# YiwenShaoStephen/mergeNet

Hardware: AMD Instinct MI355X
Metric: merged Mpixels/sec at 1024x2048 (speculative fast path; proven path: value_proven_path) (higher is better)
Workload: dtype f32

## Files before the change

### include/mergenet_hip.h

```cpp
#ifndef MERGENET_HIP_H_
#define MERGENET_HIP_H_

#include <stddef.h>
#include <stdint.h>

#ifdef __cplusplus
extern "C" {
#endif

#define MN_MAX_OFFSETS 32
#define MN_MAX_CLASSES 127

enum mn_status {
  MN_OK = 0,
  MN_ERR_ARGUMENT = -1,
  MN_ERR_OFFSETS = -2,
  MN_ERR_NO_DEVICE = -3,
  MN_ERR_CAPACITY = -4,
  MN_ERR_NO_BACKGROUND = -10,
  MN_ERR_INTERNAL = -20,
  MN_ERR_UNPROVEN = -30
};

enum mn_variant {
// ... 92 lines not shown
int mn_segment_finish(mn_context* ctx, mn_stats* stats);

int mn_sweep_time_device(mn_context* ctx, const float* const* d_class_pred, const float* const* d_adj_pred,
                         int n_inputs, int class_dim, int offset_dim, int img_width, int img_height,
                         int num_classes, const int* offset_list, const mn_options* opts, void* stream, int reps,
                         float* us_per_launch);

int mn_segment_exact_batch(mn_context** ctxs, int count, const float* const* d_class_pred, int class_dim,
                           const float* const* d_adj_pred, int offset_dim, int img_width, int img_height,
                           int num_classes, const int* offset_list, int* const* d_mask,
                           int* const* d_object_class, int* const* d_partition, const mn_options* opts,
                           void* stream, mn_stats* stats);

int mn_score_device(mn_context* ctx, const float* d_class_pred, int class_dim,
                    const float* d_adj_pred, int offset_dim, int img_width, int img_height,
                    int num_classes, const int* offset_list, const mn_options* opts, void* stream,
                    unsigned char* d_cls_out, unsigned long long* d_best_out, float* ms_class_pass,
                    float* ms_edge_pass);

int mn_sweep_device(mn_context* ctx, const float* d_class_pred, int class_dim, const float* d_adj_pred,
                    int offset_dim, int img_width, int img_height, int num_classes, const int* offset_list,
                    const mn_options* opts, void* stream, unsigned* d_bits_out, float* d_neg_out,
                    unsigned char* d_cls_out, int* d_gsum_out, double* logsum_out, int* info_out);

int mn_exact_phase_a_device(mn_context* ctx, const float* d_class_pred, int class_dim,
                            const float* d_adj_pred, int offset_dim, int img_width, int img_height,
                            int num_classes, const int* offset_list, const mn_options* opts, void* stream,
                            unsigned char* d_cls_out, float* d_oml_out, float* d_prio_out);

int mn_segment_device_t(mn_context* ctx, const void* d_class_pred, int class_dim, const void* d_adj_pred,
                        int offset_dim, int dtype, int img_width, int img_height, int num_classes,
                        const int* offset_list, int* d_mask, int* d_object_class, int* d_partition,
                        const mn_options* opts, void* stream, mn_stats* stats);
int mn_segment_launch_t(mn_context* ctx, const void* d_class_pred, int class_dim, const void* d_adj_pred,
                        int offset_dim, int dtype, int img_width, int img_height, int num_classes,
                        const int* offset_list, int* d_mask, int* d_object_class, int* d_partition,
                        const mn_options* opts, void* stream);
int mn_segment_exact_batch_t(mn_context** ctxs, int count, const void* const* d_class_pred, int class_dim,
                             const void* const* d_adj_pred, int offset_dim, int dtype, int img_width,
                             int img_height, int num_classes, const int* offset_list, int* const* d_mask,
                             int* const* d_object_class, int* const* d_partition, const mn_options* opts,
                             void* stream, mn_stats* stats);
int mn_score_device_t(mn_context* ctx, const void* d_class_pred, int class_dim, const void* d_adj_pred,
                      int offset_dim, int dtype, int img_width, int img_height, int num_classes,
                      const int* offset_list, const mn_options* opts, void* stream, unsigned char* d_cls_out,
                      unsigned long long* d_best_out, float* ms_class_pass, float* ms_edge_pass);
// ... 68 lines not shown
```

### mergenet_amd/csrc/mergenet_hip.hip

```cpp
#include <hip/hip_runtime.h>
#include <hip/hip_ext.h>

#include <math.h>
#include <stdio.h>
#include <stdlib.h>
#include <string.h>
#include <time.h>

#include "../../include/mergenet_hip.h"
#include "mn_device.h"
#include "mn_kernels_score.h"
#include "mn_kernels_merge.h"
#include "mn_kernels_finish.h"
#include "mn_kernels_output.h"
#include "mn_kernels_prepare.h"
#include "mn_kernels_cc.h"
#include "mn_kernels_tail.h"
#include "mn_kernels_exact.h"
#include "mn_kernels_reforder.h"

#define MN_NSCALARS 16
#define MN_STAT_BYTES ((((sizeof(Counters) + 15) & ~(size_t)15)) + MN_NSCALARS * sizeof(int) + 4 * sizeof(double))

#define MN_MAX_SUBROUNDS 64
// ... 61 lines not shown
  HashTab T;
  int* block_count;
  double* partial;
  Counters* cnt;
  int* scalars;
  unsigned* gmax;
  unsigned* touch;
  unsigned* h_touch;
  float* theta;
  int* progress;
  u64* bg_key;
  double* lp_out;
  Counters* h_cnt;
  int* h_scalars;
  double* h_lp;
  size_t cc_sum_lds, oc_lds;
  unsigned char* statblk;
  unsigned char* h_statblk;
  int *cc_tcount, *cc_lcount;
  unsigned* cc_bits;
  int* cc_roots;
  int cc_sign_blocks;
  unsigned* cc_negbits;
  size_t cc_cap_max;
  hipEvent_t ev[12];
  struct Pending {
    int active;
    int rc;
    Queued queued;
    ImageCall call;
    mn_stats stats;
  } pend;
  hipEvent_t ev_done;
  struct Replay {
    int state;
    int capturing;
    unsigned char key[256];
    size_t key_bytes;
    hipGraph_t gA, gB;
    hipGraphExec_t eA, eB;
    hipStream_t cap;
    Queued queued;
  } replay;
  hipStream_t side;
  hipEvent_t ev_fork;
  ImgParams last_params;
// ... 289 lines not shown
  if (hipSetDevice(device) != hipSuccess) { g_last_status = MN_ERR_NO_DEVICE; return NULL; }
  mn_context* c = static_cast<mn_context*>(calloc(1, sizeof(mn_context)));
  if (!c) { g_last_status = MN_ERR_INTERNAL; return NULL; }
  c->device = device;
  c->maxH = max_height; c->maxW = max_width; c->maxC = max_classes; c->maxO = max_offsets;
  c->N = (size_t)max_height * max_width;
  c->Rmax = c->N * (size_t)max_offsets;
  c->cap_full = next_pow2(c->Rmax + c->Rmax / 4 + 1024);
  if (ctx_alloc(c) != MN_OK) { mn_destroy(c); return NULL; }
  g_last_status = MN_OK;
  return c;
}

extern "C" void mn_destroy(mn_context* c) {
  if (!c) return;
  if (getenv("MN_TRACE_HOST") && g_host_n[1] > 0) {
    fprintf(stderr, "host: %lld launches %.1f us each; %lld read-backs: waiting for the image %.1f us, the rest %.1f us each\n",
            g_host_n[0], g_host_us[0] / (double)(g_host_n[0] ? g_host_n[0] : 1), g_host_n[1],
            g_host_us[1] / (double)g_host_n[1], g_host_us[2] / (double)g_host_n[1]);
    g_host_n[0] = g_host_n[1] = 0; g_host_us[0] = g_host_us[1] = g_host_us[2] = 0.0;
  }
  (void)hipSetDevice(c->device);
  void* dev[] = {c->ocls, c->cls0, c->lpvalid, c->matched, c->pruned, c->osize, c->parent, c->mate, c->root,
                 c->label, c->mapbuf, c->lpsum, c->lp_acc, c->ball, c->bsub, c->fin_lists, c->cc_tcount, c->cc_lcount, c->cc_bits, c->cc_roots, c->cc_negbits,
                 c->block_count, c->wire_counts, c->partial, c->statblk,
                 c->bg_key, c->gmax, c->touch, c->theta, c->progress, c->d_class, c->d_same, c->d_mask, c->d_objcls, c->d_part};
  for (size_t i = 0; i < sizeof(dev) / sizeof(dev[0]); i++)
    if (dev[i]) (void)hipFree(dev[i]);
  x_free(c);
  r_free(c);
  if (c->xw.d_P) (void)hipFree(c->xw.d_P);
  if (c->xw.d_X) (void)hipFree(c->xw.d_X);
  if (c->rw.d_S) (void)hipFree(c->rw.d_S);
  free_records(c);
  if (c->h_statblk) (void)hipHostFree(c->h_statblk);
  if (c->h_touch) (void)hipHostFree(c->h_touch);
  for (int i = 0; i < 12; i++)
    if (c->ev[i]) (void)hipEventDestroy(c->ev[i]);
  if (c->ev_done) (void)hipEventDestroy(c->ev_done);
  if (c->ev_fork) (void)hipEventDestroy(c->ev_fork);
  if (c->side) (void)hipStreamDestroy(c->side);
  if (c->replay.eA) (void)hipGraphExecDestroy(c->replay.eA);
  if (c->replay.eB) (void)hipGraphExecDestroy(c->replay.eB);
  if (c->replay.gA) (void)hipGraphDestroy(c->replay.gA);
  if (c->replay.gB) (void)hipGraphDestroy(c->replay.gB);
  if (c->replay.cap) (void)hipStreamDestroy(c->replay.cap);
  free(c);
}

extern "C" size_t mn_workspace_bytes(const mn_context* c) { return c ? c->bytes : 0; }

static int ensure_fast(mn_context* c) {
  if (c->lp_acc) return MN_OK;
  const size_t N = c->N;
  MN_HIP(dev_alloc(c, &c->lp_acc, N * (size_t)c->maxC));
  MN_HIP(dev_alloc(c, &c->ball, N));
  MN_HIP(dev_alloc(c, &c->bsub, N));
  MN_HIP(dev_alloc(c, &c->cc_bits, N));
  MN_HIP(dev_alloc(c, &c->cc_roots, N));
  MN_HIP(dev_alloc(c, &c->cc_negbits, N + 16));
  return MN_OK;
}

static void drop_replay_graphs(mn_context::Replay& rp) {
  if (rp.eA) { (void)hipGraphExecDestroy(rp.eA); rp.eA = nullptr; }
  if (rp.eB) { (void)hipGraphExecDestroy(rp.eB); rp.eB = nullptr; }
  if (rp.gA) { (void)hipGraphDestroy(rp.gA); rp.gA = nullptr; }
  if (rp.gB) { (void)hipGraphDestroy(rp.gB); rp.gB = nullptr; }
  rp.state = 0;
}

static int ensure_general(mn_context* c) {
  if (c->gen_ready) return MN_OK;
  MN_HIP(hipDeviceSynchronize());
  free_records(c);
  if (alloc_records(c, c->cap_full) != MN_OK) return MN_ERR_NO_DEVICE;
  c->cap = c->cap_full;
  c->gen_ready = 1;
  c->cc_clean = 0;
  drop_replay_graphs(c->replay);
  return MN_OK;
}

static int check_args(const mn_context* c, const ImageCall& call) {
  const int W = call.W, H = call.H, num_classes = call.num_classes, offset_dim = call.offset_dim;
  const int* offs = call.offs;
  if (!c || !call.has_offsets) return MN_ERR_ARGUMENT;
  if (W <= 0 || H <= 0 || num_classes <= 0 || offset_dim <= 0 || call.class_dim < num_classes)
    return MN_ERR_ARGUMENT;
  if (num_classes > MN_MAX_CLASSES || offset_dim > MN_MAX_OFFSETS) return MN_ERR_ARGUMENT;
  if ((size_t)W * H > c->N || num_classes > c->maxC || offset_dim > c->maxO) return MN_ERR_CAPACITY;
  if (call.opts.variant != MN_VARIANT_CSEGMENT && call.opts.variant != MN_VARIANT_PYSEGMENTER)
// ... 245 lines not shown
  } while (0)
  if (P.dtype == MN_DTYPE_F32) {
    if (px == 4) launch_sign<4, MN_DTYPE_F32>(c, P, st, cls, lean_cls);
    else launch_sign<1, MN_DTYPE_F32>(c, P, st, false, false);
  } else if (px == 8) MN_SWEEP_DT(8);
  else if (px == 4) MN_SWEEP_DT(4);
  else { cls = false; lean_cls = false; MN_SWEEP_DT(1); }
#undef MN_SWEEP_DT
}

template <int PX>
static void launch_cc_hook(mn_context* c, const ImgParams& P, hipStream_t st, unsigned kmask,
                           const unsigned* hook_bits = nullptr, hipEvent_t hook_done = nullptr) {
  const int N = P.N, ngroups = (N + PX - 1) / PX;
  const dim3 gx(8 * ((grid_for(ngroups, 256) + 7) / 8));
  if (hook_done)
    hipExtLaunchKernelGGL(mn_cc_hook<PX>, gx, dim3(256), 0, st, nullptr, hook_done, 0, P,
                          hook_bits ? hook_bits : (const unsigned*)c->cc_bits, c->parent, kmask);
  else
    hipLaunchKernelGGL(mn_cc_hook<PX>, gx, dim3(256), 0, st, P, hook_bits ? hook_bits : (const unsigned*)c->cc_bits,
                       c->parent, kmask);
}

enum CcUse {
  CC_WAITED,
  CC_QUEUED_COMPACT,
  CC_QUEUED_TAIL,
  CC_CORES
};

static int run_components(mn_context* c, const ImgParams& P, hipStream_t& st, CcUse use) {
  const bool wait = use == CC_WAITED, with_ball = use == CC_WAITED;
  const bool with_compact = use == CC_WAITED || use == CC_QUEUED_COMPACT;
  const bool fork_before_sums = use == CC_QUEUED_TAIL, cores = use == CC_CORES;
  const int N = P.N;
  ObjState S = obj_state(c);
  const dim3 b(256);
  const bool four = P.W % 4 == 0;
  int kh = -1, kv = -1, dv = 0;
  for (int k = 0; k < P.O; k++) {
    if (kh < 0 && P.di[k] == 0 && P.dj[k] == 1) kh = k;
    if (kv < 0 && P.dj[k] == 0 && (P.di[k] == 1 || P.di[k] == -1)) { kv = k; dv = P.di[k]; }
  }
  const bool few_events = (c->debug_flags & 2) != 0;
  const bool lean = (c->debug_flags & 16) != 0;
  const dim3 tiles((P.W + 63) / 64, (P.H + MN_CC_TILE_ROWS - 1) / MN_CC_TILE_ROWS);
  const int px = sweep_px(c, P);
  const bool sweep4 = px >= 4;
  const size_t sign_blocks = grid_for((size_t)(N / px), MN_CC_SIGN_THREADS);
  c->cc_sign_blocks = (int)(sign_blocks * (MN_CC_SIGN_THREADS / 64));
  int* clsmin = c->root;
  int* clsmax = c->mapbuf;
  const bool fused_cls = sweep4;
  const bool lean_cls = fused_cls && !cores;
  launch_sweep(c, P, st, px, fused_cls, lean_cls);
  if (!few_events && !c->ext_events) MN_HIP(hipEventRecord(c->ev[10], st));
  const unsigned* lbits = c->cc_bits;
  unsigned kshort = 0u;
  if (cores) {
    if (!fused_cls) {
      const unsigned blocks = grid_for((size_t)(N >> 2) > 0 ? (size_t)(N >> 2) : 1, 256);
      hipLaunchKernelGGL(mn_class_pass, dim3(blocks), dim3(256), 0, st, P, c->cls0);
    }
    unsigned* bits2 = reinterpret_cast<unsigned*>(c->label);
    for (int k = 0; k < P.O; k++)
      if (c->core_radius < 0 || (abs(P.di[k]) <= c->core_radius && abs(P.dj[k]) <= c->core_radius)) kshort |= 1u << k;
    hipLaunchKernelGGL(mn_core_clean, dim3(grid_for(N, 256)), b, 0, st, P, (const unsigned*)c->cc_bits,
                       (const unsigned char*)c->cls0, c->pruned, kshort);
    hipLaunchKernelGGL(mn_core_bits, dim3(grid_for(N, 256)), b, 0, st, P, (const unsigned char*)c->pruned,
                       (const unsigned*)c->cc_bits, (const unsigned char*)c->cls0, bits2);
    lbits = bits2;
  }
  hipStream_t real = st;
  if (c->replay.capturing) {
    MN_HIP(hipStreamBeginCapture(c->replay.cap, hipStreamCaptureModeThreadLocal));
    st = c->replay.cap;
  }
  unsigned kmask = P.O >= 32 ? 0xFFFFFFFFu : ((1u << P.O) - 1u);
  const bool fork_ext = fork_before_sums && c->ext_events && !c->replay.capturing;
  bool fork_by_hook = false;
  hipLaunchKernelGGL(mn_cc_tiles, tiles, dim3(MN_CC_TILE_ROWS * 64), 0, st, P, lbits, c->parent, kh, kv, dv,
                     c->osize, c->lp_acc, clsmin, clsmax, c->matched);
  if (kh >= 0 || kv >= 0) {
    hipLaunchKernelGGL(mn_cc_borders, tiles, dim3(128), 0, st, P, lbits, c->parent, kh, kv, dv);
    if (kh >= 0) kmask &= ~(1u << kh);
    if (kv >= 0) kmask &= ~(1u << kv);
  }
  hipLaunchKernelGGL(mn_cc_flatten, dim3(grid_for((size_t)(N >> 2) > 0 ? (size_t)(N >> 2) : 1, 256)), b, 0, st, N, c->parent);
  fork_by_hook = fork_ext && kmask;
  if (kmask) {
    if (four) launch_cc_hook<4>(c, P, st, kmask, lbits, fork_by_hook ? c->ev_fork : nullptr);
    else launch_cc_hook<1>(c, P, st, kmask, lbits, fork_by_hook ? c->ev_fork : nullptr);
  }
  if (c->replay.capturing) {
    MN_HIP(hipStreamEndCapture(c->replay.cap, &c->replay.gA));
    MN_HIP(hipGraphInstantiate(&c->replay.eA, c->replay.gA, nullptr, nullptr, 0));
    MN_HIP(hipGraphLaunch(c->replay.eA, real));
    st = real;
  }
  HashTab T = c->T;
  T.mask = (unsigned)(c->cc_cap - 1);
  if (!few_events && !lean) MN_HIP(hipEventRecord(c->ev[7], st));
  if (fork_before_sums) {
    if (!fork_by_hook) MN_HIP(hipEventRecord(c->ev_fork, st));
    MN_HIP(hipStreamWaitEvent(c->side, c->ev_fork, 0));
    st = c->side;
    if (c->replay.capturing) {
      MN_HIP(hipStreamBeginCapture(c->replay.cap, hipStreamCaptureModeThreadLocal));
      st = c->replay.cap;
    }
  }
  if (!few_events && !lean) MN_HIP(hipEventRecord(c->ev[11], st));
  {
    const size_t lds = (size_t)MN_CC_SUM_SLOTS * (P.C + 1) * sizeof(u64);
    if (lds > c->cc_sum_lds) {
      MN_HIP(hipFuncSetAttribute(reinterpret_cast<const void*>(mn_cc_class_sums),
// ... 1210 lines not shown
  HostBuf<double> hp(sign_waves * 2);
  if (!hp.ok()) return MN_ERR_INTERNAL;
  MN_HIP(hipMemcpyAsync(hp, c->partial, sign_waves * 2 * sizeof(double), hipMemcpyDeviceToHost, st));
  MN_HIP(hipMemcpyAsync(c->h_scalars, c->scalars, MN_NSCALARS * sizeof(int), hipMemcpyDeviceToHost, st));
  MN_HIP(hipStreamSynchronize(st));
  double t = 0.0;
  for (size_t b = 0; b < sign_waves; b++) t += hp[2 * b];
  if (logsum_out) *logsum_out = t;
  if (info_out) { info_out[0] = px; info_out[1] = fused_cls ? 1 : 0; info_out[2] = c->h_scalars[6]; }
  MN_HIP(hipGetLastError());
  g_last_status = MN_OK;
  return MN_OK;
}

extern "C" int mn_sweep_device(mn_context* c, const float* d_class_pred, int class_dim,
                               const float* d_adj_pred, int offset_dim, int W, int H, int num_classes,
                               const int* offset_list, const mn_options* opts, void* stream,
                               unsigned* d_bits_out, float* d_neg_out, unsigned char* d_cls_out,
                               int* d_gsum_out, double* logsum_out, int* info_out) {
  return mn_sweep_device_t(c, d_class_pred, class_dim, d_adj_pred, offset_dim, MN_DTYPE_F32, W, H, num_classes,
                           offset_list, opts, stream, d_bits_out, d_neg_out, d_cls_out, d_gsum_out, logsum_out, info_out);
}

extern "C" int mn_sweep_time_device_t(mn_context* c, const void* const* d_class_pred, const void* const* d_adj_pred,
                                      int dtype, int n_inputs, int class_dim, int offset_dim, int W, int H,
                                      int num_classes, const int* offset_list, const mn_options* opts, void* stream,
                                      int reps, float* us_per_launch) {
  const bool ok = d_class_pred && d_adj_pred && n_inputs >= 1 && reps >= 1 && us_per_launch;
  ImageCall call = {ok ? d_class_pred[0] : nullptr, ok ? d_adj_pred[0] : nullptr, dtype, class_dim, offset_dim, W, H, num_classes};
  image_call(&call, offset_list, opts, stream);
  ImgParams P;
  const int rc = begin_call(c, call, ok, nullptr, &P);
  if (rc != MN_OK) return rc;
  hipStream_t st = static_cast<hipStream_t>(stream);
  if (ensure_fast(c) != MN_OK) return MN_ERR_NO_DEVICE;
  c->debug_flags = call.opts.debug_flags | 2;
  c->ext_events = 0;
  c->cc_clean = 0;
  MN_HIP(hipMemsetAsync(c->scalars, 0, MN_NSCALARS * sizeof(int), st));
  for (int phase = 0; phase < 2; phase++) {
    const int n = phase == 0 ? (reps + 9) / 10 : reps;
    if (phase == 1) MN_HIP(hipEventRecord(c->ev[0], st));
    for (int i = 0; i < n; i++) {
      call.d_class = d_class_pred[i % n_inputs]; call.d_adj = d_adj_pred[i % n_inputs];
      fill_params(&P, call);
      launch_sweep(c, P, st, sweep_px(c, P), true, true);
// ... 372 lines not shown
```

### mergenet_amd/csrc/mn_kernels_cc.h

```cpp
#pragma once

static_assert(MN_MAX_OFFSETS <= 32, "edge masks are 32-bit words: one bit per offset");

#include "mn_device.h"
#include "mn_kernels_merge.h"

#define MN_LP_FIX 16777216.0

__device__ __forceinline__ int mn_cc_find(int* __restrict__ parent, int x) {
  int p = parent[x];
  while (p != x) {
    const int g = parent[p];
    if (g != p) parent[x] = g;
    x = p;
    p = g;
  }
  return x;
}

struct __attribute__((packed, aligned(4))) mn_int4u { int x, y, z, w; };
__device__ __forceinline__ int4 mn_ld_int4_unaligned(const int* __restrict__ p) {
  const mn_int4u t = *reinterpret_cast<const mn_int4u*>(p);
  return make_int4(t.x, t.y, t.z, t.w);
}
// ... 363 lines not shown

__device__ __forceinline__ void mn_cc_wave_union(int* __restrict__ parent, bool want, int a, int b) {
  const int lane = threadIdx.x & 63;
  u64 todo = __ballot(want);
  const u64 key = mn_key(a, b);
  while (todo) {
    const int first = __ffsll((long long)todo) - 1;
    const u64 k0v = ((u64)(unsigned)__shfl((int)(key >> 32), first) << 32) |
                    (u64)(unsigned)__shfl((int)(key & 0xFFFFFFFFull), first);
    const bool mine = want && key == k0v;
    if (lane == first) {
      while (a != b) {
        if (a < b) { const int t = a; a = b; b = t; }
        const int old = atomicMin(&parent[a], b);
        if (old == a) break;
        a = mn_cc_find(parent, old);
        b = mn_cc_find(parent, b);
      }
    }
    todo &= ~__ballot(mine);
  }
}

__global__ __launch_bounds__(128) void mn_cc_borders(ImgParams P, const unsigned* __restrict__ bits,
                                                     int* __restrict__ parent, int kh, int kv, int dv) {
  const int lane = threadIdx.x & 63, wave = threadIdx.x >> 6;
  const int r0 = (int)blockIdx.y * MN_CC_TILE_ROWS, c0 = (int)blockIdx.x * 64;
  int p = -1, q = -1;
  if (wave == 0) {
    const int r = r0 + lane, c = c0 + 63;
    if (kh >= 0 && lane < MN_CC_TILE_ROWS && r < P.H && c + 1 < P.W) {
      p = r * P.W + c;
      if ((bits[p] >> kh) & 1u) q = p + 1;
    }
  } else {
    const int r = dv > 0 ? r0 + MN_CC_TILE_ROWS - 1 : r0, c = c0 + lane;
    if (kv >= 0 && r < P.H && r + dv >= 0 && r + dv < P.H && c < P.W) {
      p = r * P.W + c;
      if ((bits[p] >> kv) & 1u) q = p + dv * P.W;
    }
  }
  int a = 0, b = 0;
  bool want = false;
  if (q >= 0) {
    a = mn_cc_find(parent, p);
    b = mn_cc_find(parent, q);
    want = a != b;
  }
  mn_cc_wave_union(parent, want, a, b);
}

__global__ __launch_bounds__(256) void mn_cc_flatten(int N, int* __restrict__ parent) {
  const int i = blockIdx.x * blockDim.x + threadIdx.x;
  const int n4 = N >> 2;
  if (i < n4) {
    int4 r = *reinterpret_cast<const int4*>(parent + 4 * (size_t)i);
    int4 o = r;
    int x = r.x; while (parent[x] != x) x = parent[x]; o.x = x;
    if (r.y == r.x) o.y = o.x; else { x = r.y; while (parent[x] != x) x = parent[x]; o.y = x; }
    if (r.z == r.x) o.z = o.x; else { x = r.z; while (parent[x] != x) x = parent[x]; o.z = x; }
    if (r.w == r.x) o.w = o.x; else { x = r.w; while (parent[x] != x) x = parent[x]; o.w = x; }
    if (o.x != r.x || o.y != r.y || o.z != r.z || o.w != r.w)
      *reinterpret_cast<int4*>(parent + 4 * (size_t)i) = o;
  }
  if (i < N - (n4 << 2)) {
    const int p = (n4 << 2) + i;
    int x = p; while (parent[x] != x) x = parent[x];
    parent[p] = x;
  }
}

template <int PX>
// ... 46 lines not shown
      }
    }
#pragma unroll
    for (int g = 0; g < G; g++) {
      const int k = k0 + g;
      if (k >= P.O) break;
      if (__ballot((any >> k) & 1u) == 0) continue;
#pragma unroll
      for (int j = 0; j < PX; j++) {
        bool want = false;
        int a = 0, bb = 0;
        if (((b[j] & kmask) >> k) & 1u) {
          if (rq[g][j] != own[j]) {
            const int q = p0 + j + P.di[k] * P.W + P.dj[k];
            a = mn_cc_find(parent, p0 + j);
            bb = mn_cc_find(parent, q);
            want = a != bb;
          }
        }
        mn_cc_wave_union(parent, want, a, bb);
      }
    }
  }
}

__global__ __launch_bounds__(256) void mn_core_clean(ImgParams P, const unsigned* __restrict__ bits,
                                                     const unsigned char* __restrict__ cls0,
                                                     unsigned char* __restrict__ clean, unsigned kshort) {
  const int p = blockIdx.x * blockDim.x + threadIdx.x;
  if (p >= P.N) return;
  const int r = p / P.W, c = p - r * P.W;
  const unsigned b = bits[p];
  const unsigned char mine = cls0[p];
  bool ok = true;
  for (int k = 0; k < P.O; k++) {
    if (!((kshort >> k) & 1u)) continue;
    const int di = P.di[k], dj = P.dj[k];
    if (r + di >= 0 && r + di < P.H && c + dj >= 0 && c + dj < P.W) {
      const int q = p + di * P.W + dj;
      ok = ok && ((b >> k) & 1u) && cls0[q] == mine;
    }
    if (r - di >= 0 && r - di < P.H && c - dj >= 0 && c - dj < P.W) {
      const int q = p - di * P.W - dj;
      ok = ok && ((bits[q] >> k) & 1u) && cls0[q] == mine;
    }
  }
// ... 675 lines not shown
```

### mergenet_amd/segmenter.py

```python

from __future__ import annotations

import ctypes
import os
import threading
from collections import namedtuple
from typing import List, Optional, Sequence, Tuple

import numpy as np

_HERE = os.path.dirname(os.path.abspath(__file__))
LIB_PATH = os.environ.get("MN_LIB") or os.path.join(_HERE, "libmergenet_hip.so")

MN_VARIANT_CSEGMENT = 0
MN_VARIANT_PYSEGMENTER = 1
MN_MODE_AUTO, MN_MODE_EXACT, MN_MODE_ROUNDS, MN_MODE_COMPONENTS = 0, 1, 2, 3
MN_ERR_NO_BACKGROUND = -10
MN_ERR_UNPROVEN = -30
MN_DEBUG_GENERIC_EDGE_PASS, MN_DEBUG_NO_EVENTS, MN_DEBUG_NO_CORES = 1, 2, 4
MN_DEBUG_LEAN_EVENTS, MN_DEBUG_REPLAY = 16, 32
MN_DEBUG_SWEEP16_4PX = 256
MN_DTYPE_F32, MN_DTYPE_F16, MN_DTYPE_BF16 = 0, 1, 2
MN_ERR_ARGUMENT = -1
MN_PROVE_ALWAYS, MN_PROVE_BY_MODE, MN_PROVE_NEVER = 1, 0, -1
# ... 21 lines not shown
                ("num_instances", ctypes.c_int), ("num_objects", ctypes.c_int),
                ("rounds", ctypes.c_int), ("finisher_steps", ctypes.c_int),
                ("cert_edge_violations", ctypes.c_int),
                ("cert_class_violations", ctypes.c_int), ("cert_record_violations", ctypes.c_int),
                ("initial_records", ctypes.c_longlong),
                ("merges", ctypes.c_longlong), ("total_logprob", ctypes.c_double),
                ("ms_score", ctypes.c_float), ("ms_class_pass", ctypes.c_float),
                ("ms_edge_pass", ctypes.c_float), ("ms_merge", ctypes.c_float),
                ("ms_output", ctypes.c_float), ("ms_total", ctypes.c_float),
                ("ms_cc_label", ctypes.c_float), ("ms_cc_sums", ctypes.c_float),
                ("ms_cc_edges", ctypes.c_float), ("ms_cc_cross", ctypes.c_float),
                ("proof", ctypes.c_int), ("cores_condemned", ctypes.c_int), ("tied_steps", ctypes.c_int), ("tied_merges", ctypes.c_int),
                ("tie_order_used", ctypes.c_int), ("tied_conflicts", ctypes.c_int)]

    def as_dict(self) -> dict:
        return {name: getattr(self, name) for name, _ in self._fields_ if name != "reserved_i"}


_f32p = ctypes.POINTER(ctypes.c_float)
_i32p = ctypes.POINTER(ctypes.c_int)
_lib_handle = None

EXPORTS = ["mn_default_options", "mn_create", "mn_destroy", "mn_workspace_bytes",
           "mn_segment_device", "mn_segment_launch", "mn_segment_finish", "mn_segment_exact_batch", "mn_score_device", "mn_exact_phase_a_device", "mn_sweep_device", "mn_sweep_time_device", "mn_segment_host", "c_run_segmentation",
           "mn_prepare_device", "mn_upsample_mask_device", "mn_rle_points_device", "mn_rle_encode_host", "mn_sameness_targets_device", "mn_instance_scores_device",
           "mn_pack_wire_device", "mn_runs_wire_words", "mn_pack_runs_device", "mn_unpack_runs_device",
           "mn_unpack_runs_batch_device",
           "mn_segment_device_t", "mn_segment_launch_t", "mn_segment_exact_batch_t", "mn_score_device_t",
           "mn_exact_phase_a_device_t", "mn_sweep_device_t", "mn_sweep_time_device_t", "mn_prepare_device_t",
           "mn_last_status", "mn_status_string", "mn_version"]


def load_library() -> ctypes.CDLL:
    global _lib_handle
    if _lib_handle is not None:
        return _lib_handle
    if not os.path.exists(LIB_PATH):
        raise RuntimeError("HIP extension missing: %s (run __graft_entry__.build() / make -C "
                           "mergenet_amd/csrc); there is no CPU fallback" % LIB_PATH)
    try:
        import torch
    except ImportError:
        pass
    lib = ctypes.CDLL(LIB_PATH)
    lib.mn_default_options.argtypes = [ctypes.POINTER(MnOptions)]
    lib.mn_default_options.restype = None
    lib.mn_create.argtypes = [ctypes.c_int] * 5
# ... 17 lines not shown
                                           ctypes.c_int, ctypes.c_int, _i32p, _vpp, _vpp, _vpp,
                                           ctypes.POINTER(MnOptions), ctypes.c_void_p, ctypes.POINTER(MnStats)]
    lib.mn_segment_exact_batch.restype = ctypes.c_int
    if hasattr(lib, "mn_sweep_time_device"):
        lib.mn_sweep_time_device.argtypes = [ctypes.c_void_p, _vpp, _vpp, ctypes.c_int, ctypes.c_int, ctypes.c_int,
                                             ctypes.c_int, ctypes.c_int, ctypes.c_int, _i32p,
                                             ctypes.POINTER(MnOptions), ctypes.c_void_p, ctypes.c_int, _f32p]
        lib.mn_sweep_time_device.restype = ctypes.c_int
    lib.mn_score_device.argtypes = [ctypes.c_void_p, ctypes.c_void_p, ctypes.c_int, ctypes.c_void_p,
                                    ctypes.c_int, ctypes.c_int, ctypes.c_int, ctypes.c_int, _i32p,
                                    ctypes.POINTER(MnOptions), ctypes.c_void_p, ctypes.c_void_p,
                                    ctypes.c_void_p, _f32p, _f32p]
    lib.mn_score_device.restype = ctypes.c_int
    lib.mn_exact_phase_a_device.argtypes = [ctypes.c_void_p, ctypes.c_void_p, ctypes.c_int, ctypes.c_void_p,
                                            ctypes.c_int, ctypes.c_int, ctypes.c_int, ctypes.c_int, _i32p,
                                            ctypes.POINTER(MnOptions), ctypes.c_void_p, ctypes.c_void_p,
                                            ctypes.c_void_p, ctypes.c_void_p]
    lib.mn_exact_phase_a_device.restype = ctypes.c_int
    lib.mn_sweep_device.argtypes = [ctypes.c_void_p, ctypes.c_void_p, ctypes.c_int, ctypes.c_void_p, ctypes.c_int,
                                    ctypes.c_int, ctypes.c_int, ctypes.c_int, _i32p, ctypes.POINTER(MnOptions),
                                    ctypes.c_void_p, ctypes.c_void_p, ctypes.c_void_p, ctypes.c_void_p,
                                    ctypes.c_void_p, ctypes.POINTER(ctypes.c_double), _i32p]
    lib.mn_sweep_device.restype = ctypes.c_int
    lib.mn_segment_host.argtypes = [ctypes.c_void_p, _f32p, ctypes.c_int, _f32p, ctypes.c_int,
                                    ctypes.c_int, ctypes.c_int, ctypes.c_int, _i32p, _i32p, _i32p,
                                    _i32p, ctypes.POINTER(MnOptions), ctypes.POINTER(MnStats)]
    lib.mn_segment_host.restype = ctypes.c_int
    lib.c_run_segmentation.argtypes = [_f32p, ctypes.c_int, _f32p, ctypes.c_int, ctypes.c_int,
                                       ctypes.c_int, ctypes.c_int, _i32p, _i32p, _i32p,
                                       ctypes.c_float, ctypes.c_float, ctypes.c_float]
    lib.c_run_segmentation.restype = None
    lib.mn_prepare_device.argtypes = [ctypes.c_void_p, ctypes.c_void_p, ctypes.c_int, ctypes.c_int,
                                      ctypes.c_int, ctypes.c_void_p, ctypes.c_int, ctypes.c_int,
                                      ctypes.c_int, ctypes.c_int, ctypes.c_void_p]
    lib.mn_prepare_device.restype = ctypes.c_int
    if hasattr(lib, "mn_segment_device_t"):
        def typed(argtypes, at=5):
            return list(argtypes[:at]) + [ctypes.c_int] + list(argtypes[at:])
        lib.mn_segment_device_t.argtypes = typed(lib.mn_segment_device.argtypes)
        lib.mn_segment_launch_t.argtypes = typed(lib.mn_segment_launch.argtypes)
        lib.mn_segment_exact_batch_t.argtypes = typed(lib.mn_segment_exact_batch.argtypes, 6)
        lib.mn_score_device_t.argtypes = typed(lib.mn_score_device.argtypes)
        lib.mn_exact_phase_a_device_t.argtypes = typed(lib.mn_exact_phase_a_device.argtypes)
        lib.mn_sweep_device_t.argtypes = typed(lib.mn_sweep_device.argtypes)
        lib.mn_sweep_time_device_t.argtypes = typed(lib.mn_sweep_time_device.argtypes, 3)
        lib.mn_prepare_device_t.argtypes = [ctypes.c_void_p, ctypes.c_void_p, ctypes.c_int, ctypes.c_int, ctypes.c_int,
# ... 351 lines not shown
    def sweep(self, class_probs, same_probs, offsets, opts: Optional[MnOptions] = None):
        torch = self.torch
        C, H, W, O, off = self._check(class_probs, same_probs, offsets)
        opts = opts if opts is not None else default_options()
        dev = class_probs.device
        bits = torch.empty((H, W), dtype=torch.int32, device=dev)
        neg = torch.empty((O, H, W), dtype=torch.float32, device=dev)
        cls = torch.zeros((H, W), dtype=torch.uint8, device=dev)
        gsum = torch.zeros((C, (H * W + 3) // 4), dtype=torch.int32, device=dev)
        logsum = ctypes.c_double(0.0)
        info = (ctypes.c_int * 3)()
        stream = torch.cuda.current_stream(dev).cuda_stream
        fn, dt = self._typed("mn_sweep_device", self._dtype(class_probs))
        rc = fn(self.handle, class_probs.data_ptr(), C, same_probs.data_ptr(), O, *dt, W, H, C,
                off.ctypes.data_as(_i32p), ctypes.byref(opts), ctypes.c_void_p(stream),
                bits.data_ptr(), neg.data_ptr(), cls.data_ptr(), gsum.data_ptr(),
                ctypes.byref(logsum), info)
        if rc != 0:
            raise MergeNetError(rc)
        fused = bool(info[1])
        return dict(bits=bits, neg=neg, cls=cls if fused else None, gsum=gsum if fused else None,
                    logsum=logsum.value, pixels_per_lane=int(info[0]), fused_class=fused, margin_edges=int(info[2]))

    def sweep_time(self, inputs: Sequence, offsets, opts: Optional[MnOptions] = None, reps: int = 400) -> float:
        for a, b in inputs:
            C, H, W, O, off = self._check(a, b, offsets)
            if a.dtype != inputs[0][0].dtype or a.shape != inputs[0][0].shape:
                raise ValueError("the input sets of a sweep timing share one dtype and shape")
        opts = opts if opts is not None else default_options()
        n = len(inputs)
        vp = ctypes.c_void_p * n
        out = ctypes.c_float(0)
        stream = self.torch.cuda.current_stream(inputs[0][0].device).cuda_stream
        fn, dt = self._typed("mn_sweep_time_device", self._dtype(inputs[0][0]))
        rc = fn(self.handle, vp(*[a.data_ptr() for a, _ in inputs]),
                vp(*[b.data_ptr() for _, b in inputs]), *dt, n, C, O, W, H, C,
                off.ctypes.data_as(_i32p), ctypes.byref(opts), ctypes.c_void_p(stream),
                int(reps), ctypes.byref(out))
        if rc != 0:
            raise MergeNetError(rc)
        return out.value

    def exact_phase_a(self, class_probs, same_probs, offsets, opts: Optional[MnOptions] = None):
        torch = self.torch
        C, H, W, O, off = self._check(class_probs, same_probs, offsets)
        opts = opts if opts is not None else default_options()
# ... 335 lines not shown
```

Before: 16130.

## Add four-pixel-per-lane tile labelling with border records for CC

Adds a tile labelling kernel for images whose width is a multiple of four. Each lane loads four pixels with one 16-byte read, resolves horizontal runs with wave ballots and shuffles, and performs the vertical unions in shared memory. Each tile writes its edge roots to a small record buffer, so a new border kernel can join neighbouring tiles by reading records instead of re-reading the bit image. The labelling sequence is factored into a shared helper, and a new debug entry point (mn_label_bits_device) exposes it. The cost is an extra device buffer and more kernel code, which could lower occupancy.

```diff
diff --git a/include/mergenet_hip.h b/include/mergenet_hip.h
--- a/include/mergenet_hip.h
+++ b/include/mergenet_hip.h
@@ -138,6 +138,9 @@
                     int offset_dim, int img_width, int img_height, int num_classes, const int* offset_list,
                     const mn_options* opts, void* stream, unsigned* d_bits_out, float* d_neg_out,
                     unsigned char* d_cls_out, int* d_gsum_out, double* logsum_out, int* info_out);
+
+int mn_label_bits_device(mn_context* ctx, const unsigned* d_bits, int img_width, int img_height, int offset_dim,
+                         const int* offset_list, void* stream, int* d_root_out, unsigned char* d_cand_out);
 
 int mn_exact_phase_a_device(mn_context* ctx, const float* d_class_pred, int class_dim,
                             const float* d_adj_pred, int offset_dim, int img_width, int img_height,
diff --git a/mergenet_amd/csrc/mergenet_hip.hip b/mergenet_amd/csrc/mergenet_hip.hip
--- a/mergenet_amd/csrc/mergenet_hip.hip
+++ b/mergenet_amd/csrc/mergenet_hip.hip
@@ -107,6 +107,8 @@
   int* cc_roots;
   int cc_sign_blocks;
   unsigned* cc_negbits;
+  int* cc_brec;
+  size_t cc_brec_cap;
   size_t cc_cap_max;
   hipEvent_t ev[12];
   struct Pending {
@@ -442,7 +444,7 @@
   }
   (void)hipSetDevice(c->device);
   void* dev[] = {c->ocls, c->cls0, c->lpvalid, c->matched, c->pruned, c->osize, c->parent, c->mate, c->root,
-                 c->label, c->mapbuf, c->lpsum, c->lp_acc, c->ball, c->bsub, c->fin_lists, c->cc_tcount, c->cc_lcount, c->cc_bits, c->cc_roots, c->cc_negbits,
+                 c->label, c->mapbuf, c->lpsum, c->lp_acc, c->ball, c->bsub, c->fin_lists, c->cc_tcount, c->cc_lcount, c->cc_bits, c->cc_roots, c->cc_negbits, c->cc_brec,
                  c->block_count, c->wire_counts, c->partial, c->statblk,
                  c->bg_key, c->gmax, c->touch, c->theta, c->progress, c->d_class, c->d_same, c->d_mask, c->d_objcls, c->d_part};
   for (size_t i = 0; i < sizeof(dev) / sizeof(dev[0]); i++)
@@ -488,6 +490,28 @@
   if (rp.gA) { (void)hipGraphDestroy(rp.gA); rp.gA = nullptr; }
   if (rp.gB) { (void)hipGraphDestroy(rp.gB); rp.gB = nullptr; }
   rp.state = 0;
+}
+
+static size_t brec_ints(int W, int H) {
+  return (size_t)((W + MN_CC_TILE_COLS - 1) / MN_CC_TILE_COLS) * (size_t)((H + MN_CC_TILE_ROWS - 1) / MN_CC_TILE_ROWS) *
+         MN_CC_REC_INTS;
+}
+static int ensure_brec(mn_context* c, int W, int H) {
+  size_t need = brec_ints(W, H);
+  if (need <= c->cc_brec_cap) return MN_OK;
+  const size_t whole = brec_ints(c->maxW, c->maxH);
+  if (need < whole) need = whole;
+  if (c->cc_brec) {
+    MN_HIP(hipDeviceSynchronize());
+    (void)hipFree(c->cc_brec);
+    c->cc_brec = nullptr;
+    c->bytes -= (c->cc_brec_cap * sizeof(int) + 255) & ~(size_t)255;
+    c->cc_brec_cap = 0;
+    drop_replay_graphs(c->replay);
+  }
+  MN_HIP(dev_alloc(c, &c->cc_brec, need));
+  c->cc_brec_cap = need;
+  return MN_OK;
 }
 
 static int ensure_general(mn_context* c) {
@@ -779,6 +803,41 @@
                        c->parent, kmask);
 }
 
+static bool launch_labelling(mn_context* c, const ImgParams& P, hipStream_t st, const unsigned* lbits, hipEvent_t fork_ev) {
+  const int N = P.N;
+  const bool four = P.W % 4 == 0;
+  int kh = -1, kv = -1, dv = 0;
+  for (int k = 0; k < P.O; k++) {
+    if (kh < 0 && P.di[k] == 0 && P.dj[k] == 1) kh = k;
+    if (kv < 0 && P.dj[k] == 0 && (P.di[k] == 1 || P.di[k] == -1)) { kv = k; dv = P.di[k]; }
+  }
+  int* clsmin = c->root;
+  int* clsmax = c->mapbuf;
+  unsigned kmask = P.O >= 32 ? 0xFFFFFFFFu : ((1u << P.O) - 1u);
+  if (four) {
+    const dim3 tiles((P.W + MN_CC_TILE_COLS - 1) / MN_CC_TILE_COLS, (P.H + MN_CC_TILE_ROWS - 1) / MN_CC_TILE_ROWS);
+    hipLaunchKernelGGL(mn_cc_tiles4, tiles, dim3(MN_CC_TILE_ROWS * MN_CC_TILE_COLS / 4), 0, st, P, lbits, c->parent, kh, kv, dv,
+                       c->osize, c->lp_acc, clsmin, clsmax, c->matched, c->cc_brec);
+    if (kh >= 0 || kv >= 0)
+      hipLaunchKernelGGL(mn_cc_borders_rec, tiles, dim3(64 + MN_CC_TILE_COLS), 0, st, c->parent, (const int*)c->cc_brec, kh, kv, dv);
+  } else {
+    const dim3 tiles((P.W + 63) / 64, (P.H + MN_CC_TILE_ROWS - 1) / MN_CC_TILE_ROWS);
+    hipLaunchKernelGGL(mn_cc_tiles, tiles, dim3(MN_CC_TILE_ROWS * 64), 0, st, P, lbits, c->parent, kh, kv, dv,
+                       c->osize, c->lp_acc, clsmin, clsmax, c->matched);
+    if (kh >= 0 || kv >= 0)
+      hipLaunchKernelGGL(mn_cc_borders, tiles, dim3(128), 0, st, P, lbits, c->parent, kh, kv, dv);
+  }
+  if (kh >= 0) kmask &= ~(1u << kh);
+  if (kv >= 0) kmask &= ~(1u << kv);
+  hipLaunchKernelGGL(mn_cc_flatten, dim3(grid_for((size_t)(N >> 2) > 0 ? (size_t)(N >> 2) : 1, 256)), dim3(256), 0, st, N, c->parent);
+  const bool fork_by_hook = fork_ev && kmask;
+  if (kmask) {
+    if (four) launch_cc_hook<4>(c, P, st, kmask, lbits, fork_by_hook ? fork_ev : nullptr);
+    else launch_cc_hook<1>(c, P, st, kmask, lbits, fork_by_hook ? fork_ev : nullptr);
+  }
+  return fork_by_hook;
+}
+
 enum CcUse {
   CC_WAITED,
   CC_QUEUED_COMPACT,
@@ -793,15 +852,12 @@
   const int N = P.N;
   ObjState S = obj_state(c);
   const dim3 b(256);
-  const bool four = P.W % 4 == 0;
-  int kh = -1, kv = -1, dv = 0;
-  for (int k = 0; k < P.O; k++) {
-    if (kh < 0 && P.di[k] == 0 && P.dj[k] == 1) kh = k;
-    if (kv < 0 && P.dj[k] == 0 && (P.di[k] == 1 || P.di[k] == -1)) { kv = k; dv = P.di[k]; }
-  }
   const bool few_events = (c->debug_flags & 2) != 0;
   const bool lean = (c->debug_flags & 16) != 0;
-  const dim3 tiles((P.W + 63) / 64, (P.H + MN_CC_TILE_ROWS - 1) / MN_CC_TILE_ROWS);
+  {
+    const int rc = ensure_brec(c, P.W, P.H);
+    if (rc != MN_OK) return rc;
+  }
   const int px = sweep_px(c, P);
   const bool sweep4 = px >= 4;
   const size_t sign_blocks = grid_for((size_t)(N / px), MN_CC_SIGN_THREADS);
@@ -833,22 +889,8 @@
     MN_HIP(hipStreamBeginCapture(c->replay.cap, hipStreamCaptureModeThreadLocal));
     st = c->replay.cap;
   }
-  unsigned kmask = P.O >= 32 ? 0xFFFFFFFFu : ((1u << P.O) - 1u);
   const bool fork_ext = fork_before_sums && c->ext_events && !c->replay.capturing;
-  bool fork_by_hook = false;
-  hipLaunchKernelGGL(mn_cc_tiles, tiles, dim3(MN_CC_TILE_ROWS * 64), 0, st, P, lbits, c->parent, kh, kv, dv,
-                     c->osize, c->lp_acc, clsmin, clsmax, c->matched);
-  if (kh >= 0 || kv >= 0) {
-    hipLaunchKernelGGL(mn_cc_borders, tiles, dim3(128), 0, st, P, lbits, c->parent, kh, kv, dv);
-    if (kh >= 0) kmask &= ~(1u << kh);
-    if (kv >= 0) kmask &= ~(1u << kv);
-  }
-  hipLaunchKernelGGL(mn_cc_flatten, dim3(grid_for((size_t)(N >> 2) > 0 ? (size_t)(N >> 2) : 1, 256)), b, 0, st, N, c->parent);
-  fork_by_hook = fork_ext && kmask;
-  if (kmask) {
-    if (four) launch_cc_hook<4>(c, P, st, kmask, lbits, fork_by_hook ? c->ev_fork : nullptr);
-    else launch_cc_hook<1>(c, P, st, kmask, lbits, fork_by_hook ? c->ev_fork : nullptr);
-  }
+  const bool fork_by_hook = launch_labelling(c, P, st, lbits, fork_ext ? c->ev_fork : nullptr);
   if (c->replay.capturing) {
     MN_HIP(hipStreamEndCapture(c->replay.cap, &c->replay.gA));
     MN_HIP(hipGraphInstantiate(&c->replay.eA, c->replay.gA, nullptr, nullptr, 0));
@@ -2105,6 +2147,31 @@
                            offset_list, opts, stream, d_bits_out, d_neg_out, d_cls_out, d_gsum_out, logsum_out, info_out);
 }
 
+extern "C" int mn_label_bits_device(mn_context* c, const unsigned* d_bits, int W, int H, int offset_dim,
+                                    const int* offset_list, void* stream, int* d_root_out, unsigned char* d_cand_out) {
+  ImageCall call = {nullptr, nullptr, MN_DTYPE_F32, 1, offset_dim, W, H, 1};
+  image_call(&call, offset_list, nullptr, stream);
+  int rc = check_args(c, call);
+  if (rc == MN_OK && (!d_bits || !d_root_out || !d_cand_out)) rc = MN_ERR_ARGUMENT;
+  if (rc != MN_OK) { g_last_status = rc; return rc; }
+  MN_HIP(hipSetDevice(c->device));
+  ImgParams P;
+  fill_params(&P, call);
+  hipStream_t st = call.stream;
+  const int N = P.N;
+  if (ensure_fast(c) != MN_OK) return MN_ERR_NO_DEVICE;
+  if ((rc = ensure_brec(c, W, H)) != MN_OK) return rc;
+  c->cc_clean = 0;
+  hipLaunchKernelGGL(mn_cc_import_bits, dim3(grid_for((size_t)N, 256)), dim3(256), 0, st, P, d_bits, c->cc_bits);
+  (void)launch_labelling(c, P, st, c->cc_bits, nullptr);
+  hipLaunchKernelGGL(mn_cc_export_roots, dim3(grid_for((size_t)N, 256)), dim3(256), 0, st, N, (const int*)c->parent, d_root_out);
+  MN_HIP(hipMemcpyAsync(d_cand_out, c->matched, (size_t)N, hipMemcpyDeviceToDevice, st));
+  MN_HIP(hipStreamSynchronize(st));
+  MN_HIP(hipGetLastError());
+  g_last_status = MN_OK;
+  return MN_OK;
+}
+
 extern "C" int mn_sweep_time_device_t(mn_context* c, const void* const* d_class_pred, const void* const* d_adj_pred,
                                       int dtype, int n_inputs, int class_dim, int offset_dim, int W, int H,
                                       int num_classes, const int* offset_list, const mn_options* opts, void* stream,
diff --git a/mergenet_amd/csrc/mn_kernels_cc.h b/mergenet_amd/csrc/mn_kernels_cc.h
--- a/mergenet_amd/csrc/mn_kernels_cc.h
+++ b/mergenet_amd/csrc/mn_kernels_cc.h
@@ -409,6 +409,102 @@
   }
 }
 
+#ifndef MN_CC_TILE_COLS
+#define MN_CC_TILE_COLS 64
+#endif
+static_assert(MN_CC_TILE_COLS == 64 || MN_CC_TILE_COLS == 256, "a tile row is a quarter or the whole of a wave");
+static_assert(MN_CC_TILE_ROWS >= 2 && MN_CC_TILE_ROWS * MN_CC_TILE_COLS / 4 <= 1024 && (MN_CC_TILE_ROWS * MN_CC_TILE_COLS / 4) % 64 == 0,
+              "mn_cc_tiles4: one block of whole waves per tile");
+#define MN_CC_REC_RIGHT 0
+#define MN_CC_REC_FIRSTCOL MN_CC_TILE_ROWS
+#define MN_CC_REC_LEAVE (2 * MN_CC_TILE_ROWS)
+#define MN_CC_REC_FACE (2 * MN_CC_TILE_ROWS + MN_CC_TILE_COLS)
+#define MN_CC_REC_INTS (2 * MN_CC_TILE_ROWS + 2 * MN_CC_TILE_COLS)
+static_assert(MN_CC_TILE_ROWS % 4 == 0, "the record sections are read and written as 16-byte words");
+
+__global__ __launch_bounds__(MN_CC_TILE_ROWS * MN_CC_TILE_COLS / 4) void mn_cc_tiles4(
+    ImgParams P, const unsigned* __restrict__ bits, int* __restrict__ parent, int kh, int kv, int dv,
+    int* __restrict__ osize, i64* __restrict__ lp_acc, int* __restrict__ clsmin, int* __restrict__ clsmax,
+    unsigned char* __restrict__ cand, int* __restrict__ rec) {
+  constexpr int TW = MN_CC_TILE_COLS, LPR = TW / 4;
+  __shared__ __attribute__((aligned(16))) int lab[MN_CC_TILE_ROWS * TW];
+  const int t = threadIdx.x, lane = t & 63, l = t % LPR, i = t / LPR;
+  const int r = (int)blockIdx.y * MN_CC_TILE_ROWS + i, c0 = (int)blockIdx.x * TW + 4 * l;
+  const bool in = r < P.H && c0 < P.W;
+  const int p0 = in ? r * P.W + c0 : 0;
+  unsigned b[4] = {0u, 0u, 0u, 0u};
+  if (in) {
+    const uint4 q = *reinterpret_cast<const uint4*>(bits + p0);
+    b[0] = q.x; b[1] = q.y; b[2] = q.z; b[3] = q.w;
+  }
+  const unsigned hbit = kh >= 0 ? 1u << kh : 0u, vbit = kv >= 0 ? 1u << kv : 0u;
+  const bool h0 = b[0] & hbit, h1 = b[1] & hbit, h2 = b[2] & hbit;
+  const bool h3 = (b[3] & hbit) && l < LPR - 1;
+  const int exit = h3 ? 4 * l + (!h2 ? 3 : !h1 ? 2 : !h0 ? 1 : 0) : 4 * (l + 1);
+  const u64 through = __ballot(h0 && h1 && h2 && h3);
+  const u64 lower = (lane ? ((1ull << lane) - 1ull) : 0ull) & ~((1ull << (lane - l)) - 1ull);
+  const u64 below = ~through & lower;
+  const int from = __shfl(exit, below ? 63 - __clzll((long long)below) : lane);
+  int s[4];
+  s[0] = below ? from : 0;
+  s[1] = h0 ? s[0] : 4 * l + 1;
+  s[2] = h1 ? s[1] : 4 * l + 2;
+  s[3] = h2 ? s[2] : 4 * l + 3;
+  const int base = i * TW;
+  *reinterpret_cast<int4*>(&lab[base + 4 * l]) = make_int4(base + s[0], base + s[1], base + s[2], base + s[3]);
+  __syncthreads();
+  const int ni = i + dv;
+  const bool vrow = kv >= 0 && ni >= 0 && ni < MN_CC_TILE_ROWS;
+  bool want[4];
+  int ua[4], ub[4];
+#pragma unroll
+  for (int j = 0; j < 4; j++) { want[j] = vrow && (b[j] & vbit); ua[j] = base + s[j]; ub[j] = 0; }
+  if (want[0] || want[1] || want[2] || want[3]) {
+    const int4 q = *reinterpret_cast<const int4*>(&lab[ni * TW + 4 * l]);
+    ub[0] = q.x; ub[1] = q.y; ub[2] = q.z; ub[3] = q.w;
+  }
+  const bool same1 = want[0] && ua[1] == ua[0] && ub[1] == ub[0];
+  const bool same2 = want[1] && ua[2] == ua[1] && ub[2] == ub[1];
+  const bool same3 = want[2] && ua[3] == ua[2] && ub[3] == ub[2];
+  mn_cc_wave_union(lab, want[0], ua[0], ub[0]);
+  mn_cc_wave_union(lab, want[1] && !same1, ua[1], ub[1]);
+  mn_cc_wave_union(lab, want[2] && !same2, ua[2], ub[2]);
+  mn_cc_wave_union(lab, want[3] && !same3, ua[3], ub[3]);
+  __syncthreads();
+  int root[4];
+#pragma unroll
+  for (int j = 0; j < 4; j++) {
+    if (j > 0 && s[j] == s[j - 1]) { root[j] = root[j - 1]; continue; }
+    int x = base + s[j];
+    while (lab[x] != x) x = lab[x];
+    root[j] = in ? ((int)blockIdx.y * MN_CC_TILE_ROWS + (int)((unsigned)x / TW)) * P.W + (int)blockIdx.x * TW + (int)((unsigned)x % TW) : -1;
+  }
+  int* __restrict__ R = rec + ((size_t)blockIdx.y * gridDim.x + blockIdx.x) * MN_CC_REC_INTS;
+  if (l == LPR - 1) R[MN_CC_REC_RIGHT + i] = (b[3] & hbit) ? root[3] : -1;
+  if (l == 0) R[MN_CC_REC_FIRSTCOL + i] = root[0];
+  if (dv != 0) {
+    if (i == (dv > 0 ? MN_CC_TILE_ROWS - 1 : 0))
+      *reinterpret_cast<int4*>(&R[MN_CC_REC_LEAVE + 4 * l]) =
+          make_int4((b[0] & vbit) ? root[0] : -1, (b[1] & vbit) ? root[1] : -1, (b[2] & vbit) ? root[2] : -1,
+                    (b[3] & vbit) ? root[3] : -1);
+    if (i == (dv > 0 ? 0 : MN_CC_TILE_ROWS - 1))
+      *reinterpret_cast<int4*>(&R[MN_CC_REC_FACE + 4 * l]) = make_int4(root[0], root[1], root[2], root[3]);
+  }
+  if (!in) return;
+  *reinterpret_cast<int4*>(parent + p0) = make_int4(root[0], root[1], root[2], root[3]);
+  uchar4 isroot;
+  isroot.x = root[0] == p0; isroot.y = root[1] == p0 + 1; isroot.z = root[2] == p0 + 2; isroot.w = root[3] == p0 + 3;
+  *reinterpret_cast<uchar4*>(cand + p0) = isroot;
+#pragma unroll
+  for (int j = 0; j < 4; j++)
+    if (root[j] == p0 + j) {
+      osize[p0 + j] = 0;
+      for (int c = 0; c < P.C; c++) lp_acc[(size_t)c * P.N + p0 + j] = 0;
+      clsmin[p0 + j] = 255;
+      clsmax[p0 + j] = 0;
+    }
+}
+
 __global__ __launch_bounds__(128) void mn_cc_borders(ImgParams P, const unsigned* __restrict__ bits,
                                                      int* __restrict__ parent, int kh, int kv, int dv) {
   const int lane = threadIdx.x & 63, wave = threadIdx.x >> 6;
@@ -435,6 +531,26 @@
     want = a != b;
   }
   mn_cc_wave_union(parent, want, a, b);
+}
+
+__global__ __launch_bounds__(64 + MN_CC_TILE_COLS) void mn_cc_borders_rec(int* __restrict__ parent,
+                                                                        const int* __restrict__ rec, int kh, int kv, int dv) {
+  const int t = threadIdx.x;
+  const int* __restrict__ R = rec + ((size_t)blockIdx.y * gridDim.x + blockIdx.x) * MN_CC_REC_INTS;
+  int a = -1, b = -1;
+  if (t < 64) {
+    if (kh >= 0 && t < MN_CC_TILE_ROWS && blockIdx.x + 1 < gridDim.x) {
+      a = R[MN_CC_REC_RIGHT + t];
+      b = R[MN_CC_REC_INTS + MN_CC_REC_FIRSTCOL + t];
+    }
+  } else {
+    const int nby = (int)blockIdx.y + dv;
+    if (kv >= 0 && dv != 0 && nby >= 0 && nby < (int)gridDim.y) {
+      a = R[MN_CC_REC_LEAVE + t - 64];
+      b = (R + (long long)dv * (long long)gridDim.x * MN_CC_REC_INTS)[MN_CC_REC_FACE + t - 64];
+    }
+  }
+  mn_cc_wave_union(parent, a >= 0 && b >= 0 && a != b, a, b);
 }
 
 __global__ __launch_bounds__(256) void mn_cc_flatten(int N, int* __restrict__ parent) {
@@ -527,6 +643,27 @@
       }
     }
   }
+}
+
+__global__ __launch_bounds__(256) void mn_cc_import_bits(ImgParams P, const unsigned* __restrict__ src,
+                                                         unsigned* __restrict__ bits) {
+  const int p = blockIdx.x * 256 + threadIdx.x;
+  if (p >= P.N) return;
+  const int r = p / P.W, c = p - r * P.W;
+  unsigned ok = 0u;
+  for (int k = 0; k < P.O; k++) {
+    const int rr = r + P.di[k], cc = c + P.dj[k];
+    if (rr >= 0 && rr < P.H && cc >= 0 && cc < P.W) ok |= 1u << k;
+  }
+  bits[p] = src[p] & ok;
+}
+
+__global__ __launch_bounds__(256) void mn_cc_export_roots(int N, const int* __restrict__ parent, int* __restrict__ out) {
+  const int p = blockIdx.x * 256 + threadIdx.x;
+  if (p >= N) return;
+  int x = p;
+  while (parent[x] != x) x = parent[x];
+  out[p] = x;
 }
 
 __global__ __launch_bounds__(256) void mn_core_clean(ImgParams P, const unsigned* __restrict__ bits,
diff --git a/mergenet_amd/segmenter.py b/mergenet_amd/segmenter.py
--- a/mergenet_amd/segmenter.py
+++ b/mergenet_amd/segmenter.py
@@ -67,7 +67,7 @@
 _lib_handle = None
 
 EXPORTS = ["mn_default_options", "mn_create", "mn_destroy", "mn_workspace_bytes",
-           "mn_segment_device", "mn_segment_launch", "mn_segment_finish", "mn_segment_exact_batch", "mn_score_device", "mn_exact_phase_a_device", "mn_sweep_device", "mn_sweep_time_device", "mn_segment_host", "c_run_segmentation",
+           "mn_segment_device", "mn_segment_launch", "mn_segment_finish", "mn_segment_exact_batch", "mn_score_device", "mn_exact_phase_a_device", "mn_sweep_device", "mn_sweep_time_device", "mn_label_bits_device", "mn_segment_host", "c_run_segmentation",
            "mn_prepare_device", "mn_upsample_mask_device", "mn_rle_points_device", "mn_rle_encode_host", "mn_sameness_targets_device", "mn_instance_scores_device",
            "mn_pack_wire_device", "mn_runs_wire_words", "mn_pack_runs_device", "mn_unpack_runs_device",
            "mn_unpack_runs_batch_device",
@@ -131,6 +131,10 @@
                                     ctypes.c_void_p, ctypes.c_void_p, ctypes.c_void_p, ctypes.c_void_p,
                                     ctypes.c_void_p, ctypes.POINTER(ctypes.c_double), _i32p]
     lib.mn_sweep_device.restype = ctypes.c_int
+    if hasattr(lib, "mn_label_bits_device"):
+        lib.mn_label_bits_device.argtypes = [ctypes.c_void_p, ctypes.c_void_p, ctypes.c_int, ctypes.c_int, ctypes.c_int,
+                                             _i32p, ctypes.c_void_p, ctypes.c_void_p, ctypes.c_void_p]
+        lib.mn_label_bits_device.restype = ctypes.c_int
     lib.mn_segment_host.argtypes = [ctypes.c_void_p, _f32p, ctypes.c_int, _f32p, ctypes.c_int,
                                     ctypes.c_int, ctypes.c_int, ctypes.c_int, _i32p, _i32p, _i32p,
                                     _i32p, ctypes.POINTER(MnOptions), ctypes.POINTER(MnStats)]
@@ -528,6 +532,23 @@
         return dict(bits=bits, neg=neg, cls=cls if fused else None, gsum=gsum if fused else None,
                     logsum=logsum.value, pixels_per_lane=int(info[0]), fused_class=fused, margin_edges=int(info[2]))
 
+    def label_bits(self, bits, offsets):
+        torch = self.torch
+        if not (bits.is_cuda and bits.is_contiguous() and bits.dim() == 2 and bits.dtype == torch.int32):
+            raise ValueError("expected a contiguous int32 [H,W] tensor on the GPU")
+        if bits.device.index != self.device:
+            raise ValueError("tensor lives on another device than the Merger")
+        H, W = bits.shape
+        off = np.ascontiguousarray(np.asarray(offsets, dtype=np.int32).reshape(-1, 2))
+        root = torch.empty((H, W), dtype=torch.int32, device=bits.device)
+        cand = torch.empty((H, W), dtype=torch.uint8, device=bits.device)
+        stream = torch.cuda.current_stream(bits.device).cuda_stream
+        rc = self.lib.mn_label_bits_device(self.handle, bits.data_ptr(), W, H, len(off), off.ctypes.data_as(_i32p),
+                                           ctypes.c_void_p(stream), root.data_ptr(), cand.data_ptr())
+        if rc != 0:
+            raise MergeNetError(rc)
+        return root, cand
+
     def sweep_time(self, inputs: Sequence, offsets, opts: Optional[MnOptions] = None, reps: int = 400) -> float:
         for a, b in inputs:
             C, H, W, O, off = self._check(a, b, offsets)
```

After: 16300 (median of 6 runs). No clear change (+1.1%).
